# ZhenghaoFei/visual_odom

Measured on NVIDIA H100. Metric: stereo frames/sec at 1241x376, 2000 feats; LK kernel HBM GB/s vs roofline, higher is better.
Workload: dtype u8/i32 fixed point + f32 (LK), f64 (pose)

## Files before the change

visual_odom_b200/csrc/batch.cu:

```cuda
#include "ctx.h"
#include <string.h>
#include <algorithm>

__global__ void k_pack_counts(vo_unit_result_dev* res, const int* n_pts, const int* n_det, const int* n3, const int* n5,
                              int n_units, int detect)
{
    const int u = blockIdx.x * blockDim.x + threadIdx.x;
    if (u >= n_units) return;
    res[u].n_features = n_pts[u];
    res[u].n_detected = detect ? n_det[u] : 0;
    res[u].n_tracked = n3[u];
    res[u].n_valid = n5[u];
}

#define VO_OUT_BYTES_PER_SLOT (4 * sizeof(float2) + sizeof(int) + sizeof(float3) + sizeof(int))
__global__ void k_pack_outputs(uint8_t* __restrict__ out, size_t stride, int per, const float2* __restrict__ valid4, size_t cs,
                               const int* __restrict__ idx5, const float3* __restrict__ X, const int* __restrict__ inliers,
                               const int* __restrict__ n5, const vo_unit_result_dev* __restrict__ res, int cap)
{
    const int u = blockIdx.x;
    const int nv = min(n5[u], per), ni = min(res[u].n_inliers, per);
    float2* o4 = reinterpret_cast<float2*>(out + (size_t)u * stride);
    int* ok = reinterpret_cast<int*>(o4 + 4 * (size_t)per);
    float* oX = reinterpret_cast<float*>(ok + per);
// ... 43 lines not shown
    uint8_t* h = nullptr;
    const cudaError_t e = cudaMallocHost(&h, stride * ctx->units + 256);
    if (e != cudaSuccess) { cudaFree(q); VO_CUDA_CHECK(e); }
    if (ctx->h_out) {
        const int nu = ctx->out_units < ctx->units ? ctx->out_units : ctx->units;
        const int m = ctx->out_per < per ? ctx->out_per : per;
        for (int u = 0; u < nu; u++) {
            const PackedUnit a = packed_unit(ctx->h_out + (size_t)u * ctx->out_stride, ctx->out_per), b = packed_unit(h + (size_t)u * stride, per);
            for (int k = 0; k < 4; k++) memcpy(b.o4 + (size_t)k * per, a.o4 + (size_t)k * ctx->out_per, (size_t)m * sizeof(float2));
            memcpy(b.ok, a.ok, (size_t)m * sizeof(int));
            memcpy(b.oX, a.oX, (size_t)m * 3 * sizeof(float));
            memcpy(b.oi, a.oi, (size_t)m * sizeof(int));
        }
        cudaFreeHost(ctx->h_out);
    }
    ctx->h_out = h;
    if (ctx->d_out) {
        ctx->allocs.erase(std::find(ctx->allocs.begin(), ctx->allocs.end(), (void*)ctx->d_out));
        cudaFree(ctx->d_out);
    }
    ctx->allocs.push_back(q);
    ctx->d_out = (uint8_t*)q;
    ctx->out_units = ctx->units; ctx->out_per = per; ctx->out_stride = stride;
    return VO_OK;
}

extern "C" int vo_batch_configure(vo_ctx* ctx, int w, int h, int n_units, const float P_l[12], const float P_r[12])
{
    if (!ctx) return VO_E_INVALID;
    if (!P_l || !P_r || n_units <= 0) { vo_set_error(ctx, "bad argument"); return VO_E_INVALID; }
    VO_CUDA_CHECK(cudaSetDevice(ctx->device));
    int rc = vo_claim_buffers(ctx, "vo_batch_configure");
    if (rc) return rc;
    if ((rc = vo_ensure_state(ctx, w, h, n_units, 4))) return rc;
    vo_set_calibration(ctx, P_l, P_r);
    ctx->batch_units = n_units;
    ctx->batch_uploaded = 0;
    ctx->slot_pts.assign(n_units, 0);
    return VO_OK;
}

static int upload_range(vo_ctx* ctx, const vo_unit* units, int u0, int n, size_t pitch, cudaStream_t st, bool detect, int src0 = -1)
{
    if (src0 < 0) src0 = u0;
    const int w = ctx->w, h = ctx->h, cap = ctx->cap;
    const int total = ctx->batch_units;
    double* h_tprev = (double*)ctx->h_pinned;
    int* h_cnt = (int*)(h_tprev + 3 * (size_t)total);
    for (int u = u0; u < u0 + n; u++) {
        const vo_unit& U = units[u - u0 + src0];
        const uint8_t* imgs[4] = {U.l0, U.r0, U.l1, U.r1};
        for (int k = 0; k < 4; k++) {
            uint8_t* dst = ctx->d_raw + ((size_t)u * 4 + k) * w * h;
            if (pitch == (size_t)w) VO_CUDA_CHECK(cudaMemcpyAsync(dst, imgs[k], (size_t)w * h, cudaMemcpyHostToDevice, st));
            else VO_CUDA_CHECK(cudaMemcpy2DAsync(dst, w, imgs[k], pitch, w, h, cudaMemcpyHostToDevice, st));
        }
        if (!detect && U.n_pts > 0)
            VO_CUDA_CHECK(cudaMemcpyAsync(ctx->d_pts_in + (size_t)u * cap, U.pts, (size_t)U.n_pts * sizeof(float2),
                                          cudaMemcpyHostToDevice, st));
        h_cnt[u] = U.n_pts;
        ctx->slot_pts[u] = U.n_pts;
        for (int k = 0; k < 3; k++) h_tprev[3 * u + k] = U.t_prev[k];
    }
    VO_CUDA_CHECK(cudaMemcpyAsync(ctx->d_tprev + 3 * (size_t)u0, h_tprev + 3 * (size_t)u0, (size_t)n * 3 * sizeof(double),
                                  cudaMemcpyHostToDevice, st));
    VO_CUDA_CHECK(cudaMemcpyAsync((detect ? ctx->d_want : ctx->d_npts) + u0, h_cnt + u0, (size_t)n * sizeof(int),
                                  cudaMemcpyHostToDevice, st));
    return VO_OK;
}

static int validate_units(vo_ctx* ctx, const vo_unit* units, int n_units, size_t pitch, bool* detect_out, int* max_pts_out = nullptr)
{
    if (!ctx || !units) return VO_E_INVALID;
    if (n_units <= 0 || n_units > ctx->batch_units) { vo_set_error(ctx, "n_units=%d outside the configured batch (%d)", n_units, ctx->batch_units); return VO_E_INVALID; }
    if (pitch < (size_t)ctx->w) { vo_set_error(ctx, "pitch %zu < width %d", pitch, ctx->w); return VO_E_INVALID; }
    const bool detect = (units[0].pts == nullptr);
    int max_pts = 0;
    for (int u = 0; u < n_units; u++) {
        const vo_unit& U = units[u];
        if (!U.l0 || !U.r0 || !U.l1 || !U.r1) { vo_set_error(ctx, "unit %d: null image", u); return VO_E_INVALID; }
        if ((U.pts == nullptr) != detect) { vo_set_error(ctx, "units must all carry features or all request detection"); return VO_E_INVALID; }
        if (U.n_pts < 0 || U.n_pts > ctx->cap) { vo_set_error(ctx, "unit %d: n_pts=%d outside [0,%d]", u, U.n_pts, ctx->cap); return VO_E_CAPACITY; }
        if (U.n_pts > max_pts) max_pts = U.n_pts;
    }
    *detect_out = detect;
    if (max_pts_out) *max_pts_out = max_pts;
    const size_t bytes = (size_t)ctx->batch_units * (3 * sizeof(double) + sizeof(int) + sizeof(vo_unit_result_dev)) + 256;
    return vo_ensure_pinned(ctx, bytes);
}

static vo_unit_result_dev* pinned_results(vo_ctx* ctx)
{
    char* p = (char*)ctx->h_pinned + (size_t)ctx->batch_units * (3 * sizeof(double) + sizeof(int));
    p = (char*)(((uintptr_t)p + 63) & ~(uintptr_t)63);
    return (vo_unit_result_dev*)p;
}

extern "C" int vo_batch_upload(vo_ctx* ctx, const vo_unit* units, int n_units, size_t pitch)
{
    bool detect;
    int rc = validate_units(ctx, units, n_units, pitch, &detect);
    if (rc) return rc;
    VO_CUDA_CHECK(cudaSetDevice(ctx->device));
    if ((rc = vo_claim_buffers(ctx, "vo_batch_upload", true))) return rc;
    if ((rc = vo_drain_pending(ctx))) return rc;
    VO_CUDA_CHECK(cudaStreamSynchronize(ctx->stream));
    if ((rc = upload_range(ctx, units, 0, n_units, pitch, ctx->stream, detect))) return rc;
    ctx->batch_uploaded = n_units;
    ctx->batch_detect = detect;
    return VO_OK;
}

static int ensure_side_streams(vo_ctx* ctx)
{
    if (ctx->fork_ev) return VO_OK;
    VO_CUDA_CHECK(cudaEventCreateWithFlags(&ctx->fork_ev, cudaEventDisableTiming));
    for (int c = 0; c < VO_LANES; c++) {
        VO_CUDA_CHECK(cudaStreamCreateWithFlags(&ctx->side_stream[c], cudaStreamNonBlocking));
        VO_CUDA_CHECK(cudaEventCreateWithFlags(&ctx->join_ev[c], cudaEventDisableTiming));
    }
    return VO_OK;
}

static int ensure_hi_streams(vo_ctx* ctx)
{
    if (ctx->hi_stream[0]) return VO_OK;
    int lo = 0, hi = 0;
    VO_CUDA_CHECK(cudaDeviceGetStreamPriorityRange(&lo, &hi));
    for (int c = 0; c < VO_LANES; c++) {
        VO_CUDA_CHECK(cudaStreamCreateWithPriority(&ctx->hi_stream[c], cudaStreamNonBlocking, hi));
        for (int k = 0; k < 4; k++) VO_CUDA_CHECK(cudaEventCreateWithFlags(&ctx->hi_ev[c][k], cudaEventDisableTiming));
    }
    return VO_OK;
}

static int run_range_launch(vo_ctx* ctx, const View& v)
{
    ctx->imgs_per_unit = 4;
    int rc;
    int c = -1;
    for (int k = 0; k < VO_LANES; k++) if (ctx->side_stream[k] && v.s == ctx->side_stream[k]) c = k;
    const bool part = ctx->part_on && c >= 0;
    const bool prio = !part && ctx->use_priorities && c >= 0;
    View h = v, lk = v;
    cudaEvent_t* ev = nullptr;
    if (part) {
        h.s = ctx->part_hp_stream[c]; lk.s = ctx->part_lk_stream[c]; ev = ctx->part_ev[c];
    } else if (prio) {
        if ((rc = ensure_hi_streams(ctx))) return rc;
        h.s = ctx->hi_stream[c]; ev = ctx->hi_ev[c];
    }
    View pre = h;
    if (part && ctx->part_pre_with_lk) pre.s = lk.s;
    if (ev) {
        VO_CUDA_CHECK(cudaEventRecord(ev[0], v.s));
        VO_CUDA_CHECK(cudaStreamWaitEvent(pre.s, ev[0], 0));
        if (pre.s != h.s) VO_CUDA_CHECK(cudaStreamWaitEvent(h.s, ev[0], 0));
    }
    if (ctx->batch_detect) {
        if ((rc = vo_run_fast(ctx, pre, 0, false))) return rc;
        if ((rc = vo_run_select(ctx, pre))) return rc;
    }
    if ((rc = vo_run_pyramid(ctx, v.u0 * ctx->imgs_per_unit, v.n * ctx->imgs_per_unit, pre.s))) return rc;
    if (ev && pre.s != lk.s) {
        VO_CUDA_CHECK(cudaEventRecord(ev[1], pre.s));
        VO_CUDA_CHECK(cudaStreamWaitEvent(lk.s, ev[1], 0));
    }
    const int ip[4] = {0, 1, 3, 2}, in[4] = {1, 3, 2, 0};
    ctx->lk_per_unit = range_bound(ctx, v.u0, v.n);
    rc = vo_run_lk_ring(ctx, lk, 4, ip, in, false);
    ctx->lk_per_unit = 0;
    if (rc) return rc;
    if (ev) {
        VO_CUDA_CHECK(cudaEventRecord(ev[2], lk.s));
        VO_CUDA_CHECK(cudaStreamWaitEvent(h.s, ev[2], 0));
    }
    if ((rc = vo_run_filter(ctx, h, false))) return rc;
    const size_t cs = (size_t)ctx->units * ctx->cap;
    if ((rc = vo_run_triangulate(ctx, h, ctx->d_valid4, ctx->d_valid4 + cs, ctx->d_n5))) return rc;
    float K9[9] = {ctx->P_l[0], ctx->P_l[1], ctx->P_l[2], ctx->P_l[4], ctx->P_l[5], ctx->P_l[6], ctx->P_l[8], ctx->P_l[9], ctx->P_l[10]};
    if ((rc = vo_run_pnp(ctx, h, ctx->d_valid4 + 2 * cs, ctx->d_n5, K9))) return rc;
    k_pack_counts<<<(v.n + 63) / 64, 64, 0, h.s>>>(ctx->d_results + v.u0, ctx->d_npts + v.u0, ctx->d_ndet + v.u0, ctx->d_n3 + v.u0,
                                                  ctx->d_n5 + v.u0, v.n, ctx->batch_detect ? 1 : 0);
    ctx->launches += 1;
    VO_CUDA_CHECK(cudaGetLastError());
    if (ev) {
        VO_CUDA_CHECK(cudaEventRecord(ev[3], h.s));
        VO_CUDA_CHECK(cudaStreamWaitEvent(v.s, ev[3], 0));
    }
    return VO_OK;
}

static int run_range(vo_ctx* ctx, const View& v)
{
    bool on_side = false;
    for (int k = 0; k < VO_LANES; k++) on_side = on_side || (ctx->side_stream[k] && v.s == ctx->side_stream[k]);
    if (!ctx->use_graphs || ((ctx->use_priorities || ctx->part_on) && on_side && !ctx->batch_graphs)) return run_range_launch(ctx, v);
    const int max_pts = range_bound(ctx, v.u0, v.n);
    for (auto& g : ctx->graphs)
        if (g.u0 == v.u0 && g.n == v.n && g.detect == ctx->batch_detect && g.tma == ctx->lk_use_tma && g.s == v.s && g.max_pts == max_pts) {
            VO_CUDA_CHECK(cudaGraphLaunch(g.exec, v.s));
            ctx->launches += g.launches;
            return VO_OK;
        }
    const bool timing = ctx->lk_timing;
    const long long before = ctx->launches;
    ctx->lk_timing = false;
    cudaGraph_t graph = nullptr;
    VO_CUDA_CHECK(cudaStreamBeginCapture(v.s, cudaStreamCaptureModeThreadLocal));
    int rc = run_range_launch(ctx, v);
    cudaError_t e = cudaStreamEndCapture(v.s, &graph);
    ctx->lk_timing = timing;
    if (rc) { if (graph) cudaGraphDestroy(graph); return rc; }
    VO_CUDA_CHECK(e);
    vo_ctx::RangeGraph g;
    g.u0 = v.u0; g.n = v.n; g.detect = ctx->batch_detect; g.tma = ctx->lk_use_tma; g.s = v.s; g.max_pts = max_pts;
    g.launches = ctx->launches - before;
    VO_CUDA_CHECK(cudaGraphInstantiate(&g.exec, graph, 0));
    cudaGraphDestroy(graph);
    ctx->graphs.push_back(g);
    VO_CUDA_CHECK(cudaGraphLaunch(g.exec, v.s));
    return VO_OK;
}

extern "C" int vo_batch_run(vo_ctx* ctx)
{
    if (!ctx) return VO_E_INVALID;
    const int units = ctx->batch_uploaded;
    if (units <= 0) { vo_set_error(ctx, "vo_batch_run: nothing uploaded"); return VO_E_INVALID; }
    if (!ctx->have_P) { vo_set_error(ctx, "vo_batch_run: projection matrices not set"); return VO_E_INVALID; }
    { int rcc = vo_claim_buffers(ctx, "vo_batch_run"); if (rcc) return rcc; }
    VO_CUDA_CHECK(cudaSetDevice(ctx->device));
    if (units < 2 || ctx->batch_streams < 2) return run_range(ctx, View{0, units, ctx->stream});
    int rc = ensure_side_streams(ctx);
    if (rc) return rc;
    VO_CUDA_CHECK(cudaEventRecord(ctx->fork_ev, ctx->stream));
    const int half = (units + 1) / 2;
    for (int c = 0; c < 2; c++) {
        const int u0 = c ? half : 0, n = c ? units - half : half;
        cudaStream_t st = ctx->side_stream[c];
        VO_CUDA_CHECK(cudaStreamWaitEvent(st, ctx->fork_ev, 0));
        if ((rc = run_range(ctx, View{u0, n, st}))) return rc;
        VO_CUDA_CHECK(cudaEventRecord(ctx->join_ev[c], st));
        VO_CUDA_CHECK(cudaStreamWaitEvent(ctx->stream, ctx->join_ev[c], 0));
    }
    return VO_OK;
}

extern "C" int vo_batch_download(vo_ctx* ctx, vo_unit_result* results, int n_units)
{
    if (!ctx || !results) return VO_E_INVALID;
    if (n_units <= 0 || n_units > ctx->batch_uploaded) { vo_set_error(ctx, "n_units=%d outside the resident batch (%d)", n_units, ctx->batch_uploaded); return VO_E_INVALID; }
    static_assert(sizeof(vo_unit_result) == sizeof(vo_unit_result_dev), "result record layout");
    VO_CUDA_CHECK(cudaSetDevice(ctx->device));
    VO_CUDA_CHECK(cudaMemcpyAsync(results, ctx->d_results, (size_t)n_units * sizeof(vo_unit_result), cudaMemcpyDeviceToHost, ctx->stream));
    VO_CUDA_CHECK(cudaStreamSynchronize(ctx->stream));
    return VO_OK;
}

extern "C" int vo_frame_batch(vo_ctx* ctx, const vo_unit* units, int n_units, size_t pitch, vo_unit_result* results)
{
    bool detect;
    int rc = validate_units(ctx, units, n_units, pitch, &detect);
    if (rc) return rc;
    if (!results) return VO_E_INVALID;
    if (!ctx->have_P) { vo_set_error(ctx, "vo_frame_batch: projection matrices not set"); return VO_E_INVALID; }
    VO_CUDA_CHECK(cudaSetDevice(ctx->device));
    if ((rc = vo_claim_buffers(ctx, "vo_frame_batch", true))) return rc;
    if ((rc = vo_drain_pending(ctx))) return rc;
    VO_CUDA_CHECK(cudaStreamSynchronize(ctx->stream));
    ctx->batch_uploaded = n_units; ctx->batch_detect = detect;
    vo_unit_result_dev* h_res = pinned_results(ctx);
    const int nchunks = (n_units >= 2 && ctx->batch_streams >= 2) ? 2 : 1;
    if (nchunks == 1) {
        if ((rc = upload_range(ctx, units, 0, n_units, pitch, ctx->stream, detect))) return rc;
        if ((rc = run_range(ctx, View{0, n_units, ctx->stream}))) return rc;
        VO_CUDA_CHECK(cudaMemcpyAsync(h_res, ctx->d_results, (size_t)n_units * sizeof(vo_unit_result_dev), cudaMemcpyDeviceToHost, ctx->stream));
    } else {
        if ((rc = ensure_side_streams(ctx))) return rc;
        VO_CUDA_CHECK(cudaEventRecord(ctx->fork_ev, ctx->stream));
        const int half = (n_units + 1) / 2;
        for (int c = 0; c < 2; c++) {
            const int u0 = c ? half : 0, n = c ? n_units - half : half;
            cudaStream_t st = ctx->side_stream[c];
            VO_CUDA_CHECK(cudaStreamWaitEvent(st, ctx->fork_ev, 0));
            if ((rc = upload_range(ctx, units, u0, n, pitch, st, detect))) return rc;
            if ((rc = run_range(ctx, View{u0, n, st}))) return rc;
            VO_CUDA_CHECK(cudaMemcpyAsync(h_res + u0, ctx->d_results + u0, (size_t)n * sizeof(vo_unit_result_dev), cudaMemcpyDeviceToHost, st));
            VO_CUDA_CHECK(cudaEventRecord(ctx->join_ev[c], st));
            VO_CUDA_CHECK(cudaStreamWaitEvent(ctx->stream, ctx->join_ev[c], 0));
        }
    }
    VO_CUDA_CHECK(cudaStreamSynchronize(ctx->stream));
    memcpy(results, h_res, (size_t)n_units * sizeof(vo_unit_result));
    return VO_OK;
}

extern "C" int vo_batch_submit(vo_ctx* ctx, const vo_unit* units, int first_unit, int n_units, size_t pitch)
{
    if (!ctx) return VO_E_INVALID;
    if (first_unit < 0 || n_units <= 0 || first_unit + n_units > ctx->batch_units) {
        vo_set_error(ctx, "vo_batch_submit: slots [%d, %d) outside the configured batch (%d)", first_unit, first_unit + n_units, ctx->batch_units);
        return VO_E_INVALID;
    }
    if (!ctx->have_P) { vo_set_error(ctx, "vo_batch_submit: projection matrices not set"); return VO_E_INVALID; }
    { int rcc = vo_claim_buffers(ctx, "vo_batch_submit", true); if (rcc) return rcc; }
    for (auto& p : ctx->pending)
        if (p.active && first_unit < p.u0 + p.n && p.u0 < first_unit + n_units) {
            vo_set_error(ctx, "vo_batch_submit: slots [%d, %d) overlap a submission that has not been waited for", first_unit, first_unit + n_units);
            return VO_E_INVALID;
        }
    bool detect = ctx->batch_detect; int max_pts = 0;
    int rc;
    if (units) {
        if ((rc = validate_units(ctx, units, n_units, pitch, &detect, &max_pts))) return rc;
    } else {
        if (ctx->batch_uploaded < first_unit + n_units) {
            vo_set_error(ctx, "vo_batch_submit: units == NULL but slots [%d, %d) were never uploaded", first_unit, first_unit + n_units);
            return VO_E_INVALID;
// ... 110 lines not shown
```

visual_odom_b200/csrc/ctx.cu:

```cuda
#include "ctx.h"
#include <string.h>
#include <stdlib.h>

void vo_set_error(vo_ctx* ctx, const char* fmt, ...)
{
    if (!ctx) return;
    va_list ap;
    va_start(ap, fmt);
    vsnprintf(ctx->err, sizeof(ctx->err), fmt, ap);
    va_end(ap);
}

extern "C" void vo_default_params(vo_params* p)
{
    p->fast_threshold = 20;
    p->fast_nonmax = 1;
    p->lk_win = 21;
    p->lk_max_level = 3;
    p->lk_max_iters = 30;
    p->lk_epsilon = 0.01;
    p->lk_min_eig = 0.001;
    p->circ_threshold = 0;
    p->pnp_iterations = 500;
    p->pnp_reproj_error = 0.5f;
// ... 39 lines not shown
    VO_CUDA_CHECK(cudaStreamCreateWithFlags(&ctx->own_stream, cudaStreamNonBlocking));
    ctx->stream = ctx->own_stream;
    VO_CUDA_CHECK(vo_lk_prepare());
    ctx->cap = ctx->p.max_features;
    VO_CUDA_CHECK(cudaMalloc(&ctx->d_lk_queue, LK_QUEUES * 2 * sizeof(int)));
    VO_CUDA_CHECK(cudaMemset(ctx->d_lk_queue, 0, LK_QUEUES * 2 * sizeof(int)));
    {
        const char* st = getenv("VO_LK_STAGING");
        ctx->lk_use_tma = !(st && strcmp(st, "ldg") == 0);
        const char* sp = getenv("VO_LK_SPAN");
        if (sp) ctx->lk_span = atoi(sp);
        const char* pt = getenv("VO_SM_PARTITION");
        if (pt && atoi(pt) == 0) ctx->part_auto = false;
    }
    return VO_OK;
}

extern "C" void vo_destroy(vo_ctx* ctx)
{
    if (!ctx) return;
    cudaSetDevice(ctx->device);
    vo_drain_pending(ctx);
    if (ctx->stream) cudaStreamSynchronize(ctx->stream);
    vo_dist_shutdown(ctx);
    vo_partition_destroy(ctx);
    vo_free_state(ctx);
    for (cudaEvent_t e : ctx->ev_pool) cudaEventDestroy(e);
    for (auto& p : ctx->pending) if (p.done) cudaEventDestroy(p.done);
    for (int k = 0; k < 2; k++) {
        if (ctx->seq_front_ev[k]) cudaEventDestroy(ctx->seq_front_ev[k]);
        if (ctx->seq_back_ev[k]) cudaEventDestroy(ctx->seq_back_ev[k]);
    }
    if (ctx->fork_ev) cudaEventDestroy(ctx->fork_ev);
    for (int c = 0; c < VO_LANES; c++) {
        if (ctx->join_ev[c]) cudaEventDestroy(ctx->join_ev[c]);
        if (ctx->side_stream[c]) cudaStreamDestroy(ctx->side_stream[c]);
        if (ctx->hi_stream[c]) cudaStreamDestroy(ctx->hi_stream[c]);
        for (int k = 0; k < 4; k++) if (ctx->hi_ev[c][k]) cudaEventDestroy(ctx->hi_ev[c][k]);
    }
    if (ctx->h_pinned) cudaFreeHost(ctx->h_pinned);
    if (ctx->d_bgr) cudaFree(ctx->d_bgr);
    if (ctx->d_lk_queue) cudaFree(ctx->d_lk_queue);
    if (ctx->d_ess) cudaFree(ctx->d_ess);
    if (ctx->h_out) cudaFreeHost(ctx->h_out);
    if (ctx->own_stream) cudaStreamDestroy(ctx->own_stream);
    delete ctx;
}

extern "C" const char* vo_last_error(const vo_ctx* ctx) { return ctx ? ctx->err : "null context"; }

extern "C" int vo_set_stream(vo_ctx* ctx, void* s)
{
    if (!ctx) return VO_E_INVALID;
    VO_CUDA_CHECK(cudaStreamSynchronize(ctx->stream));
    ctx->stream = s ? (cudaStream_t)s : ctx->own_stream;
    return VO_OK;
}

extern "C" int vo_sync(vo_ctx* ctx)
{
    if (!ctx) return VO_E_INVALID;
    VO_CUDA_CHECK(cudaStreamSynchronize(ctx->stream));
    return VO_OK;
}

extern "C" int vo_set_option(vo_ctx* ctx, const char* key, double value)
{
    if (!ctx || !key) return VO_E_INVALID;
    if (strcmp(key, "batch_streams") == 0) { ctx->batch_streams = value >= 2 ? 2 : 1; return VO_OK; }
    if (strcmp(key, "lk_staging") == 0) { ctx->lk_use_tma = !(value >= 1); return VO_OK; }
    if (strcmp(key, "lk_ctas_per_sm") == 0) { ctx->lk_ctas_per_sm = (int)value; vo_drop_graphs(ctx); return VO_OK; }
    if (strcmp(key, "batch_outputs") == 0) { ctx->batch_outputs = value >= 1; vo_drop_graphs(ctx); return VO_OK; }
    if (strcmp(key, "sm_partition") == 0) {
        ctx->part_pre_with_lk = value < 0;
        ctx->part_auto = false;
        return vo_partition_enable(ctx, value < 0 ? (int)-value : (int)value);
    }
    if (strcmp(key, "lk_quota") == 0) { ctx->lk_quota = (int)value; vo_drop_graphs(ctx); return VO_OK; }
    if (strcmp(key, "lk_span") == 0) { ctx->lk_span = (int)value; vo_drop_graphs(ctx); return VO_OK; }
    if (strcmp(key, "graphs") == 0) { ctx->use_graphs = value >= 1; return VO_OK; }
    if (strcmp(key, "batch_graphs") == 0) { ctx->batch_graphs = value >= 1; return VO_OK; }
    if (strcmp(key, "priorities") == 0) { ctx->use_priorities = value >= 1; vo_drop_graphs(ctx); return VO_OK; }
    vo_set_error(ctx, "unknown option %s", key);
    return VO_E_INVALID;
}

extern "C" long long vo_kernel_launches(const vo_ctx* ctx) { return ctx ? ctx->launches : 0; }

extern "C" int vo_lk_kernel_time(vo_ctx* ctx, double* ms_total, long long* n, int reset)
{
    if (!ctx) return VO_E_INVALID;
    VO_CUDA_CHECK(cudaStreamSynchronize(ctx->stream));
    for (size_t i = 0; i + 1 < ctx->ev_used; i += 2) {
        float ms = 0.f;
        VO_CUDA_CHECK(cudaEventElapsedTime(&ms, ctx->ev_pool[i], ctx->ev_pool[i + 1]));
        ctx->lk_ms += ms;
        ctx->lk_n++;
    }
    ctx->ev_used = 0;
    if (ms_total) *ms_total = ctx->lk_ms;
    if (n) *n = ctx->lk_n;
    if (reset) { ctx->lk_ms = 0.0; ctx->lk_n = 0; }
    return VO_OK;
}

int vo_ensure_pinned(vo_ctx* ctx, size_t bytes)
{
    if (bytes <= ctx->h_pinned_bytes) return VO_OK;
    if (ctx->h_pinned) { cudaFreeHost(ctx->h_pinned); ctx->h_pinned = nullptr; ctx->h_pinned_bytes = 0; }
    VO_CUDA_CHECK(cudaMallocHost(&ctx->h_pinned, bytes));
    ctx->h_pinned_bytes = bytes;
    return VO_OK;
}

int vo_claim_buffers(vo_ctx* ctx, const char* who, bool allow_pending_batches)
{
    if (ctx->seq_inflight > 0) {
        vo_set_error(ctx, "%s: %d frame(s) submitted with vo_seq_submit have not been waited for (this call would overwrite their buffers)", who, ctx->seq_inflight);
        return VO_E_INVALID;
    }
    if (!allow_pending_batches)
        for (auto& p : ctx->pending)
            if (p.active) {
                vo_set_error(ctx, "%s: the vo_batch_submit submission of slots [%d, %d) has not been waited for", who, p.u0, p.u0 + p.n);
                return VO_E_INVALID;
            }
    ctx->seq_active = false;
    return VO_OK;
}

typedef CUresult (*PFN_cuDeviceGet)(CUdevice*, int);
typedef CUresult (*PFN_cuDeviceGetDevResource)(CUdevice, CUdevResource*, CUdevResourceType);
typedef CUresult (*PFN_cuDevSmResourceSplitByCount)(CUdevResource*, unsigned int*, const CUdevResource*, CUdevResource*, unsigned int, unsigned int);
typedef CUresult (*PFN_cuDevResourceGenerateDesc)(CUdevResourceDesc*, CUdevResource*, unsigned int);
typedef CUresult (*PFN_cuGreenCtxCreate)(CUgreenCtx*, CUdevResourceDesc, CUdevice, unsigned int);
typedef CUresult (*PFN_cuGreenCtxStreamCreate)(CUstream*, CUgreenCtx, unsigned int, int);
typedef CUresult (*PFN_cuGreenCtxDestroy)(CUgreenCtx);

template <typename F>
static bool drv(const char* name, F* fn)
{
    void* p = nullptr;
    cudaDriverEntryPointQueryResult q;
    if (cudaGetDriverEntryPoint(name, &p, cudaEnableDefault, &q) != cudaSuccess || q != cudaDriverEntryPointSuccess || !p) return false;
    *fn = (F)p;
    return true;
}

void vo_partition_destroy(vo_ctx* ctx)
{
    for (int c = 0; c < VO_LANES; c++) {
        if (ctx->part_lk_stream[c]) cudaStreamDestroy(ctx->part_lk_stream[c]);
        if (ctx->part_hp_stream[c]) cudaStreamDestroy(ctx->part_hp_stream[c]);
        ctx->part_lk_stream[c] = ctx->part_hp_stream[c] = nullptr;
        for (int k = 0; k < 4; k++) if (ctx->part_ev[c][k]) { cudaEventDestroy(ctx->part_ev[c][k]); ctx->part_ev[c][k] = nullptr; }
    }
    PFN_cuGreenCtxDestroy destroy = nullptr;
    if (drv("cuGreenCtxDestroy", &destroy))
        for (int k = 0; k < 2; k++) if (ctx->part_gctx[k]) destroy((CUgreenCtx)ctx->part_gctx[k]);
    ctx->part_gctx[0] = ctx->part_gctx[1] = nullptr;
    ctx->part_on = false; ctx->part_helper_sms = ctx->part_lk_sms = 0;
}

int vo_partition_enable(vo_ctx* ctx, int helper_sms)
{
    VO_CUDA_CHECK(cudaSetDevice(ctx->device));
    int rc = vo_drain_pending(ctx);
    if (rc) return rc;
    VO_CUDA_CHECK(cudaDeviceSynchronize());
    vo_drop_graphs(ctx);
    vo_partition_destroy(ctx);
    if (helper_sms <= 0) return VO_OK;
    PFN_cuDeviceGet dget; PFN_cuDeviceGetDevResource getres; PFN_cuDevSmResourceSplitByCount split;
    PFN_cuDevResourceGenerateDesc gendesc; PFN_cuGreenCtxCreate create; PFN_cuGreenCtxStreamCreate screate;
    if (!drv("cuDeviceGet", &dget) || !drv("cuDeviceGetDevResource", &getres) || !drv("cuDevSmResourceSplitByCount", &split) ||
        !drv("cuDevResourceGenerateDesc", &gendesc) || !drv("cuGreenCtxCreate", &create) || !drv("cuGreenCtxStreamCreate", &screate)) {
        vo_set_error(ctx, "sm_partition: this driver has no green-context API");
        return VO_E_UNSUPPORTED;
    }
    CUdevice dev;
    CUdevResource all, part[1], rest;
    unsigned int nb = 1;
    CUresult r;
    if ((r = dget(&dev, ctx->device)) != CUDA_SUCCESS || (r = getres(dev, &all, CU_DEV_RESOURCE_TYPE_SM)) != CUDA_SUCCESS ||
        (r = split(part, &nb, &all, &rest, 0, (unsigned)helper_sms)) != CUDA_SUCCESS || nb != 1) {
        vo_set_error(ctx, "sm_partition: splitting off %d SMs failed (driver error %d)", helper_sms, (int)r);
        return VO_E_UNSUPPORTED;
    }
    CUdevResource* rs[2] = {&part[0], &rest};
    for (int k = 0; k < 2; k++) {
        CUdevResourceDesc desc;
        CUgreenCtx g;
        if ((r = gendesc(&desc, rs[k], 1)) != CUDA_SUCCESS || (r = create(&g, desc, dev, CU_GREEN_CTX_DEFAULT_STREAM)) != CUDA_SUCCESS) {
            vo_set_error(ctx, "sm_partition: cuGreenCtxCreate failed (driver error %d)", (int)r);
            vo_partition_destroy(ctx);
            return VO_E_UNSUPPORTED;
        }
        ctx->part_gctx[k] = g;
    }
    ctx->part_helper_sms = (int)part[0].sm.smCount; ctx->part_lk_sms = (int)rest.sm.smCount;
    for (int c = 0; c < VO_LANES; c++) {
        CUstream a, b;
        if ((r = screate(&a, (CUgreenCtx)ctx->part_gctx[0], CU_STREAM_NON_BLOCKING, 0)) != CUDA_SUCCESS ||
            (r = screate(&b, (CUgreenCtx)ctx->part_gctx[1], CU_STREAM_NON_BLOCKING, 0)) != CUDA_SUCCESS) {
            vo_set_error(ctx, "sm_partition: cuGreenCtxStreamCreate failed (driver error %d)", (int)r);
            vo_partition_destroy(ctx);
            return VO_E_UNSUPPORTED;
        }
        ctx->part_hp_stream[c] = (cudaStream_t)a; ctx->part_lk_stream[c] = (cudaStream_t)b;
        for (int k = 0; k < 4; k++) VO_CUDA_CHECK(cudaEventCreateWithFlags(&ctx->part_ev[c][k], cudaEventDisableTiming));
    }
    ctx->part_on = true;
    return VO_OK;
}

int vo_drain_pending(vo_ctx* ctx)
{
    for (auto& p : ctx->pending)
        if (p.active) {
            VO_CUDA_CHECK(cudaEventSynchronize(p.done));
            p.active = false;
        }
    if (ctx->seq_inflight > 0 && ctx->side_stream[0]) VO_CUDA_CHECK(cudaStreamSynchronize(ctx->side_stream[0]));
    return VO_OK;
}

void vo_drop_graphs(vo_ctx* ctx)
{
    for (auto& g : ctx->graphs) cudaGraphExecDestroy(g.exec);
    ctx->graphs.clear();
}

void vo_set_calibration(vo_ctx* ctx, const float P_l[12], const float P_r[12])
{
    const bool same = ctx->have_P && memcmp(ctx->P_l, P_l, 12 * sizeof(float)) == 0 && memcmp(ctx->P_r, P_r, 12 * sizeof(float)) == 0;
    if (same) return;
    vo_drop_graphs(ctx);
    memcpy(ctx->P_l, P_l, 12 * sizeof(float));
    memcpy(ctx->P_r, P_r, 12 * sizeof(float));
    ctx->have_P = true;
}

void vo_free_state(vo_ctx* ctx)
{
    vo_drop_graphs(ctx);
    for (void* p : ctx->allocs) cudaFree(p);
    ctx->allocs.clear();
    ctx->d_out = nullptr; ctx->out_stride = 0; ctx->out_per = 0;
    ctx->w = ctx->h = ctx->units = 0;
}

template <typename T>
static cudaError_t dalloc(vo_ctx* ctx, T** p, size_t count)
{
    void* q = nullptr;
    cudaError_t e = cudaMalloc(&q, count * sizeof(T) + 256);
    if (e == cudaSuccess) { ctx->allocs.push_back(q); *p = (T*)q; }
    return e;
}

typedef CUresult (*PFN_encodeTiled)(CUtensorMap*, CUtensorMapDataType, cuuint32_t, void*, const cuuint64_t*,
                                    const cuuint64_t*, const cuuint32_t*, const cuuint32_t*, CUtensorMapInterleave,
                                    CUtensorMapSwizzle, CUtensorMapL2promotion, CUtensorMapFloatOOBfill);

static int encode_maps(vo_ctx* ctx)
{
    void* fn = nullptr;
    cudaDriverEntryPointQueryResult qres;
    VO_CUDA_CHECK(cudaGetDriverEntryPoint("cuTensorMapEncodeTiled", &fn, cudaEnableDefault, &qres));
    if (!fn || qres != cudaDriverEntryPointSuccess) {
        vo_set_error(ctx, "cuTensorMapEncodeTiled not available from the driver");
        return VO_E_CUDA;
    }
    PFN_encodeTiled enc = (PFN_encodeTiled)fn;
    const int n_img = ctx->units * 4;
    for (int l = 0; l < ctx->pg.nlevels; l++) {
        const LevelGeom& g = ctx->pg.lv[l];
        {
            cuuint64_t dims[3] = {(cuuint64_t)g.pitch, (cuuint64_t)g.hp, (cuuint64_t)n_img};
            cuuint64_t strides[2] = {(cuuint64_t)g.pitch, (cuuint64_t)g.plane};
            cuuint32_t box_i[3] = {48, 22, 1}, box_j[3] = {48, 32, 1};
            cuuint32_t estr[3] = {1, 1, 1};
            CUresult r = enc(&ctx->maps.img_i[l], CU_TENSOR_MAP_DATA_TYPE_UINT8, 3, g.img, dims, strides, box_i, estr,
                             CU_TENSOR_MAP_INTERLEAVE_NONE, CU_TENSOR_MAP_SWIZZLE_NONE,
                             CU_TENSOR_MAP_L2_PROMOTION_NONE, CU_TENSOR_MAP_FLOAT_OOB_FILL_NONE);
            if (r == CUDA_SUCCESS)
                r = enc(&ctx->maps.img_j[l], CU_TENSOR_MAP_DATA_TYPE_UINT8, 3, g.img, dims, strides, box_j, estr,
                        CU_TENSOR_MAP_INTERLEAVE_NONE, CU_TENSOR_MAP_SWIZZLE_NONE,
                        CU_TENSOR_MAP_L2_PROMOTION_NONE, CU_TENSOR_MAP_FLOAT_OOB_FILL_NONE);
            if (r != CUDA_SUCCESS) { vo_set_error(ctx, "cuTensorMapEncodeTiled(u8 level %d) failed: %d", l, (int)r); return VO_E_CUDA; }
        }
        {
            cuuint64_t dims[3] = {(cuuint64_t)g.pitch, (cuuint64_t)g.hp, (cuuint64_t)n_img};
            cuuint64_t strides[2] = {(cuuint64_t)g.pitch * 4, (cuuint64_t)g.plane * 4};
            cuuint32_t box[3] = {28, 22, 1};
            cuuint32_t estr[3] = {1, 1, 1};
            CUresult r = enc(&ctx->maps.der[l], CU_TENSOR_MAP_DATA_TYPE_UINT32, 3, g.der, dims, strides, box, estr,
                             CU_TENSOR_MAP_INTERLEAVE_NONE, CU_TENSOR_MAP_SWIZZLE_NONE,
                             CU_TENSOR_MAP_L2_PROMOTION_NONE, CU_TENSOR_MAP_FLOAT_OOB_FILL_NONE);
            if (r != CUDA_SUCCESS) { vo_set_error(ctx, "cuTensorMapEncodeTiled(deriv level %d) failed: %d", l, (int)r); return VO_E_CUDA; }
        }
    }
    return VO_OK;
}

int vo_ensure_state(vo_ctx* ctx, int w, int h, int units, int )
{
    if (w <= 0 || h <= 0 || units <= 0) { vo_set_error(ctx, "bad geometry %dx%d units=%d", w, h, units); return VO_E_INVALID; }
    if (ctx->w == w && ctx->h == h && ctx->units >= units) return VO_OK;
    VO_CUDA_CHECK(cudaSetDevice(ctx->device));
    { int drc = vo_drain_pending(ctx); if (drc) return drc; }
    VO_CUDA_CHECK(cudaStreamSynchronize(ctx->stream));
    vo_free_state(ctx);
    const int n_img = units * 4;
    const int cap = ctx->cap;
    PyrGeom& pg = ctx->pg;
    memset(&pg, 0, sizeof(pg));
    int cw = w, ch = h;
    for (int l = 0; l <= ctx->p.lk_max_level; l++) {
        if (l > 0) {
            int nw = (cw + 1) / 2, nh = (ch + 1) / 2;
            if (nw <= VO_WIN || nh <= VO_WIN) break;
            cw = nw; ch = nh;
        }
        LevelGeom& g = pg.lv[l];
        g.w = cw; g.h = ch;
        g.pitch = ((cw + 2 * VO_PAD) + 63) / 64 * 64;
        g.hp = ch + 2 * VO_PAD;
        g.plane = (size_t)g.pitch * g.hp;
        VO_CUDA_CHECK(dalloc(ctx, &g.img, g.plane * n_img));
        VO_CUDA_CHECK(dalloc(ctx, &g.der, g.plane * n_img));
        VO_CUDA_CHECK(cudaMemsetAsync(g.img, 0, g.plane * n_img, ctx->stream));
        VO_CUDA_CHECK(cudaMemsetAsync(g.der, 0, g.plane * n_img * sizeof(uint32_t), ctx->stream));
        pg.nlevels = l + 1;
    }
    pg.n_img = n_img;
    VO_CUDA_CHECK(dalloc(ctx, &ctx->d_raw, (size_t)n_img * w * h));
    VO_CUDA_CHECK(dalloc(ctx, &ctx->d_raw_tab, (size_t)n_img));
    {
        std::vector<const uint8_t*> tab(n_img);
        for (int i = 0; i < n_img; i++) tab[i] = ctx->d_raw + (size_t)i * w * h;
        VO_CUDA_CHECK(cudaMemcpyAsync(ctx->d_raw_tab, tab.data(), n_img * sizeof(uint8_t*), cudaMemcpyHostToDevice, ctx->stream));
        VO_CUDA_CHECK(cudaStreamSynchronize(ctx->stream));
    }
    const size_t uc = (size_t)units * cap;
    VO_CUDA_CHECK(dalloc(ctx, &ctx->d_pts_in, uc));
    VO_CUDA_CHECK(dalloc(ctx, &ctx->d_npts, (size_t)units));
    VO_CUDA_CHECK(dalloc(ctx, &ctx->d_pts_out, 4 * uc));
    VO_CUDA_CHECK(dalloc(ctx, &ctx->d_status, 4 * uc));
    VO_CUDA_CHECK(dalloc(ctx, &ctx->d_err, 4 * uc));
    VO_CUDA_CHECK(dalloc(ctx, &ctx->d_lk_progress, uc));
    VO_CUDA_CHECK(cudaMemsetAsync(ctx->d_lk_progress, 0, uc * sizeof(int), ctx->stream));
    VO_CUDA_CHECK(dalloc(ctx, &ctx->d_ages_in, uc));
    VO_CUDA_CHECK(dalloc(ctx, &ctx->d_ages_out, uc));
    VO_CUDA_CHECK(dalloc(ctx, &ctx->d_kept5, 5 * uc));
    VO_CUDA_CHECK(dalloc(ctx, &ctx->d_idx3, uc));
    VO_CUDA_CHECK(dalloc(ctx, &ctx->d_n3, (size_t)units));
    VO_CUDA_CHECK(dalloc(ctx, &ctx->d_valid4, 4 * uc));
    VO_CUDA_CHECK(dalloc(ctx, &ctx->d_idx5, uc));
    VO_CUDA_CHECK(dalloc(ctx, &ctx->d_n5, (size_t)units));
    {
        const long iw = w > 6 ? w - 6 : 0, ih = h > 6 ? h - 6 : 0;
        const long bound = ctx->p.fast_nonmax ? ((iw + 1) / 2) * ((ih + 1) / 2) : iw * ih;
// ... 216 lines not shown
```

visual_odom_b200/csrc/ctx.h:

```cpp
#pragma once
#include "common.cuh"
#include "lk_ring.h"
#include "filter.h"
#include "fast.h"
#include "pnp.h"
#include "seq.h"
#include "ess.h"
#include "../../include/vo_b200.h"
#include <vector>
#include <stdarg.h>
#define LK_QUEUES 32
#define VO_DIST_BUCKET 4
#define VO_DIST_NB 4
#define VO_LANES 3

struct vo_ctx {
    int device = 0;
    cudaStream_t own_stream = nullptr, stream = nullptr;
    vo_params p;
    char err[1024] = {0};
    long long launches = 0;
    int sm_count = 0;

    int w = 0, h = 0;
    int units = 0;
    int imgs_per_unit = 4;
    int cap = 0;
    PyrGeom pg;
    LkMaps maps;
    bool have_P = false;
    float P_l[12], P_r[12];

    uint8_t* d_raw = nullptr;
    const uint8_t** d_raw_tab = nullptr;
    float2* d_pts_in = nullptr;
    int* d_npts = nullptr;
    float2* d_pts_out = nullptr;
    uint8_t* d_status = nullptr;
    float* d_err = nullptr;
    int* d_ages_in = nullptr;
    int* d_ages_out = nullptr;
    float2* d_kept5 = nullptr;
    int* d_idx3 = nullptr;
    int* d_n3 = nullptr;
    float2* d_valid4 = nullptr;
    int* d_idx5 = nullptr;
    int* d_n5 = nullptr;
    uint8_t* d_score = nullptr;
    uint16_t* d_rowbuf = nullptr;
    int* d_rowcount = nullptr;
    int* d_rowoff = nullptr;
    int* d_ndet = nullptr;
    float2* d_corners = nullptr;
    float* d_resp = nullptr;
    int* d_want = nullptr;
    int corner_cap = 0;
    float3* d_X = nullptr;
    double* d_tprev = nullptr;
    PnpState* d_pnp_state = nullptr;
    int* d_subsets = nullptr;
    double* d_models = nullptr;
    int* d_counts = nullptr;
    int* d_inliers = nullptr;
    vo_unit_result_dev* d_results = nullptr;
    float2* d_feat_pts = nullptr;
    int* d_feat_ages = nullptr;
    int* d_feat_cnt = nullptr;
    int* d_bucket = nullptr;
    int* d_seq_err = nullptr;
    int feat_cap = 0, bucket_cap = 4096;
    bool seq_active = false;
    int seq_slot = 0;
    int seq_inflight = 0;
    long long seq_submitted = 0;
    int seq_channels[2] = {1, 1};
    cudaEvent_t seq_front_ev[2] = {nullptr, nullptr}, seq_back_ev[2] = {nullptr, nullptr};
    long long seq_frames = 0;
    double seq_pose[16] = {1,0,0,0, 0,1,0,0, 0,0,1,0, 0,0,0,1};
    uint8_t* d_bgr = nullptr;
    size_t bgr_bytes = 0;
    bool part_on = false;
    bool part_auto = true;
    bool part_pre_with_lk = false;
    int part_helper_sms = 0, part_lk_sms = 0;
    void* part_gctx[2] = {nullptr, nullptr};
    cudaStream_t part_lk_stream[VO_LANES] = {};
    cudaStream_t part_hp_stream[VO_LANES] = {};
    cudaEvent_t part_ev[VO_LANES][4] = {};
    void* dist_comm = nullptr;
    int dist_rank = 0, dist_world = 1;
    cudaStream_t dist_stream = nullptr, dist_snap_stream = nullptr;
    struct DistBucket { void* d = nullptr; void* h = nullptr; cudaEvent_t done = nullptr; int fill = 0, unwaited = 0, n_units = 0; bool flushed = false; };
    struct DistStep { int bucket = 0, index = 0; };
    DistBucket dist_bk[VO_DIST_NB];
    DistStep dist_steps[2 * VO_DIST_DEPTH];
    int dist_cur = 0;
    cudaEvent_t dist_ev_read = nullptr, dist_ev_fork = nullptr;
    size_t dist_bytes = 0;
    long long dist_head = 0, dist_tail = 0;
    void* d_ess = nullptr;
    int ess_cap = 0;
    std::vector<void*> allocs;

    void* h_pinned = nullptr;
    size_t h_pinned_bytes = 0;

    std::vector<cudaEvent_t> ev_pool;
    size_t ev_used = 0;
    double lk_ms = 0.0;
    long long lk_n = 0;
    bool lk_timing = true;
    bool lk_use_tma = true;
    int lk_ctas_per_sm = 0;
    int lk_quota = 0;
    int lk_span = 0;
    int* d_lk_progress = nullptr;
    int lk_per_unit = 0;
    int* d_lk_queue = nullptr;
    std::vector<cudaStream_t> lk_queue_streams;

    int batch_units = 0;
    int batch_uploaded = 0;
    bool batch_detect = false;
    int batch_streams = 2;
    bool use_graphs = true;
    struct RangeGraph { int u0, n; bool detect, tma; cudaStream_t s; int max_pts; cudaGraphExec_t exec; long long launches; };
    std::vector<RangeGraph> graphs;
    std::vector<int> slot_pts;
    cudaStream_t hi_stream[VO_LANES] = {};
    cudaEvent_t hi_ev[VO_LANES][4] = {};
    bool use_priorities = true;
    bool batch_graphs = false;
    cudaStream_t side_stream[VO_LANES] = {};
    cudaEvent_t fork_ev = nullptr, join_ev[VO_LANES] = {};
    struct Pending { int u0 = 0, n = 0; bool active = false; cudaEvent_t done = nullptr; };
    std::vector<Pending> pending;
    bool batch_outputs = false;
    uint8_t* d_out = nullptr;
    uint8_t* h_out = nullptr;
    size_t out_stride = 0;
    int out_per = 0, out_units = 0;
    unsigned submit_count = 0;
};

void vo_set_error(vo_ctx* ctx, const char* fmt, ...);
int vo_ensure_state(vo_ctx* ctx, int w, int h, int units, int imgs_per_unit);
void vo_free_state(vo_ctx* ctx);
void vo_drop_graphs(vo_ctx* ctx);
void vo_set_calibration(vo_ctx* ctx, const float P_l[12], const float P_r[12]);
int vo_drain_pending(vo_ctx* ctx);
int vo_partition_enable(vo_ctx* ctx, int helper_sms);
void vo_partition_destroy(vo_ctx* ctx);
int vo_dist_order_after_gathers(vo_ctx* ctx, cudaStream_t st);
void vo_dist_shutdown(vo_ctx* ctx);
int vo_claim_buffers(vo_ctx* ctx, const char* who, bool allow_pending_batches = false);
int vo_ensure_pinned(vo_ctx* ctx, size_t bytes);
int vo_ensure_bgr(vo_ctx* ctx, size_t bytes);
int vo_launch_bgr_to_gray(const uint8_t* d_bgr, size_t pitch, size_t img_stride_in, uint8_t* d_gray, size_t img_stride_out,
                          int w, int h, int n_img, cudaStream_t s);
struct View { int u0, n; cudaStream_t s; int plane0 = -1; };
int vo_run_lk(vo_ctx* ctx, const View& v, int ncalls, const int* img_prev, const int* img_next, bool want_err);
int vo_run_pyramid(vo_ctx* ctx, int plane0, int nplanes, cudaStream_t s);
int vo_run_lk_ring(vo_ctx* ctx, const View& v, int ncalls, const int* img_prev, const int* img_next, bool want_err);
int vo_run_filter(vo_ctx* ctx, const View& v, bool with_ages);
int vo_run_fast(vo_ctx* ctx, const View& v, int plane_in_unit, bool want_resp);
int vo_run_select(vo_ctx* ctx, const View& v);
int vo_run_triangulate(vo_ctx* ctx, const View& v, const float2* pts_l, const float2* pts_r, const int* n, float4* X4 = nullptr);
int vo_run_pnp(vo_ctx* ctx, const View& v, const float2* pts2d, const int* n, const float* K9);
```

visual_odom_b200/csrc/fast.cu:

```cuda
#include "common.cuh"
#include "fast.h"

__global__ void __launch_bounds__(256) k_fast_score(const uint8_t* const* __restrict__ img_tab, int img_stride_idx,
                                                    int w, int h, int pitch, int threshold, int nonmax,
                                                    uint8_t* __restrict__ score, size_t score_plane)
{
    constexpr int ring_dx[16] = {0, 1, 2, 3, 3, 3, 2, 1, 0, -1, -2, -3, -3, -3, -2, -1};
    constexpr int ring_dy[16] = {3, 3, 2, 1, 0, -1, -2, -3, -3, -3, -2, -1, 0, 1, 2, 3};
    const int unit = blockIdx.z;
    const uint8_t* __restrict__ img = img_tab[unit * img_stride_idx];
    uint8_t* __restrict__ sc = score + (size_t)unit * score_plane;
    const int x = blockIdx.x * 32 + (threadIdx.x & 31);
    const int y = blockIdx.y * 8 + (threadIdx.x >> 5);
    if (x >= w || y >= h) return;
    int result = 0;
    if (x >= 3 && x < w - 3 && y >= 3 && y < h - 3) {
        const uint8_t* p = img + (size_t)y * pitch + x;
        const int v = p[0];
        float d[16];
        unsigned hi = 0, lo = 0;
#pragma unroll
        for (int k = 0; k < 16; k++) {
            const int r = p[ring_dy[k] * pitch + ring_dx[k]];
            d[k] = (float)(v - r);
            hi |= (unsigned)(r > v + threshold) << k;
            lo |= (unsigned)(r < v - threshold) << k;
        }
        unsigned mh = hi | (hi << 16), ml = lo | (lo << 16);
        mh &= mh >> 1; mh &= mh >> 2; mh &= mh >> 4; mh &= mh >> 1;
        ml &= ml >> 1; ml &= ml >> 2; ml &= ml >> 4; ml &= ml >> 1;
        if (mh | ml) {
            float mn[16], mx[16];
#pragma unroll
            for (int k = 0; k < 16; k++) { mn[k] = fminf(d[k], d[(k + 1) & 15]); mx[k] = fmaxf(d[k], d[(k + 1) & 15]); }
            float mn4[16], mx4[16];
#pragma unroll
            for (int k = 0; k < 16; k++) { mn4[k] = fminf(mn[k], mn[(k + 2) & 15]); mx4[k] = fmaxf(mx[k], mx[(k + 2) & 15]); }
            float A = -1000.f, B = 1000.f;
#pragma unroll
            for (int k = 0; k < 16; k++) {
                const float a8 = fminf(mn4[k], mn4[(k + 4) & 15]);
                const float b8 = fmaxf(mx4[k], mx4[(k + 4) & 15]);
                A = fmaxf(A, fminf(a8, d[(k + 8) & 15]));
                B = fminf(B, fmaxf(b8, d[(k + 8) & 15]));
            }
            result = max(threshold, (int)fmaxf(A, -B)) - 1;
            if (!nonmax) result = 1;
        }
    }
    sc[(size_t)y * w + x] = (uint8_t)result;
}

#define NMS_T 256
#define NMS_NC 8
__global__ void __launch_bounds__(NMS_T) k_fast_nms_row(const uint8_t* __restrict__ score, size_t score_plane, int w, int h,
                                                        int nonmax, uint16_t* __restrict__ rowbuf, int rowcap,
                                                        int* __restrict__ rowcount)
{
    const int y = blockIdx.x, unit = blockIdx.y;
    const uint8_t* __restrict__ sc = score + (size_t)unit * score_plane;
    uint16_t* __restrict__ out = rowbuf + ((size_t)unit * h + y) * rowcap;
    __shared__ uint8_t rows[3][NMS_T * NMS_NC + 2];
    __shared__ int wcnt[NMS_NC * (NMS_T / 32)];
    __shared__ int base;
    if (y < 3 || y >= h - 3) {
        if (threadIdx.x == 0) rowcount[unit * h + y] = 0;
        return;
    }
    if (threadIdx.x == 0) base = 0;
    const int lane = threadIdx.x & 31, warp = threadIdx.x >> 5;
    constexpr int NW = NMS_T / 32, SPAN = NMS_T * NMS_NC;
    for (int x0 = 0; x0 < w; x0 += SPAN) {
        for (int i = threadIdx.x; i < SPAN + 2; i += NMS_T) {
            const int x = x0 - 1 + i;
            const bool in = (x >= 0 && x < w);
            rows[0][i] = in ? sc[(size_t)(y - 1) * w + x] : 0;
            rows[1][i] = in ? sc[(size_t)y * w + x] : 0;
            rows[2][i] = in ? sc[(size_t)(y + 1) * w + x] : 0;
        }
        __syncthreads();
        unsigned bal[NMS_NC];
#pragma unroll
        for (int c = 0; c < NMS_NC; c++) {
            const int x = x0 + c * NMS_T + threadIdx.x, i = c * NMS_T + threadIdx.x + 1;
            bool keep = false;
            if (x < w) {
                const int s = rows[1][i];
                if (s > 0) {
                    keep = !nonmax ||
                           (s > rows[1][i - 1] && s > rows[1][i + 1] && s > rows[0][i - 1] && s > rows[0][i] &&
                            s > rows[0][i + 1] && s > rows[2][i - 1] && s > rows[2][i] && s > rows[2][i + 1]);
                }
            }
            bal[c] = __ballot_sync(0xffffffffu, keep);
            if (lane == 0) wcnt[c * NW + warp] = __popc(bal[c]);
        }
        __syncthreads();
        int carry_total = 0;
        if (threadIdx.x < NMS_NC * NW) {
            const int v = wcnt[threadIdx.x];
            int incl = v;
#pragma unroll
            for (int d = 1; d < 32; d <<= 1) {
                const int o = __shfl_up_sync(0xffffffffu, incl, d);
                if (lane >= d) incl += o;
            }
            carry_total = incl;
            wcnt[threadIdx.x] = incl - v;
        }
        __shared__ int w0_total, pass_total;
        if (threadIdx.x == 31) w0_total = carry_total;
        __syncthreads();
        if (threadIdx.x >= 32 && threadIdx.x < NMS_NC * NW) wcnt[threadIdx.x] += w0_total;
        if (threadIdx.x == NMS_NC * NW - 1) pass_total = carry_total + w0_total;
        __syncthreads();
        const int b0 = base;
#pragma unroll
        for (int c = 0; c < NMS_NC; c++) {
            if ((bal[c] >> lane) & 1u) {
                const int o = b0 + wcnt[c * NW + warp] + __popc(bal[c] & ((1u << lane) - 1u));
                if (o < rowcap) out[o] = (uint16_t)(x0 + c * NMS_T + threadIdx.x);
            }
        }
        __syncthreads();
        if (threadIdx.x == 0) base = b0 + pass_total;
        __syncthreads();
    }
    if (threadIdx.x == 0) rowcount[unit * h + y] = base < rowcap ? base : rowcap;
}

__global__ void __launch_bounds__(1024) k_fast_scan(const int* __restrict__ rowcount, int h, int* __restrict__ rowoff,
                                                    int* __restrict__ n_det)
{
    const int unit = blockIdx.x;
    const int* rc = rowcount + unit * h;
    int* ro = rowoff + unit * h;
    __shared__ int wsum[32];
    __shared__ int carry;
    if (threadIdx.x == 0) carry = 0;
    __syncthreads();
    const int lane = threadIdx.x & 31, warp = threadIdx.x >> 5;
    for (int y0 = 0; y0 < h; y0 += 1024) {
        const int y = y0 + threadIdx.x;
        int v = (y < h) ? rc[y] : 0;
        int incl = v;
#pragma unroll
        for (int d = 1; d < 32; d <<= 1) {
            int o = __shfl_up_sync(0xffffffffu, incl, d);
            if (lane >= d) incl += o;
        }
        if (lane == 31) wsum[warp] = incl;
        __syncthreads();
        int woff = carry;
        for (int k = 0; k < warp; k++) woff += wsum[k];
        if (y < h) ro[y] = woff + incl - v;
        __syncthreads();
        if (threadIdx.x == 0) {
            int t = 0;
            for (int k = 0; k < 32; k++) t += wsum[k];
            carry += t;
        }
        __syncthreads();
    }
    if (threadIdx.x == 0) n_det[unit] = carry;
}

__global__ void __launch_bounds__(128) k_fast_gather(const uint16_t* __restrict__ rowbuf, int rowcap,
                                                     const int* __restrict__ rowcount, const int* __restrict__ rowoff,
                                                     int h, const uint8_t* __restrict__ score, size_t score_plane, int w,
                                                     int nonmax, float2* __restrict__ out, float* __restrict__ resp, int cap)
{
    const int y = blockIdx.x, unit = blockIdx.y;
    const int n = rowcount[unit * h + y], off = rowoff[unit * h + y];
    const uint16_t* src = rowbuf + ((size_t)unit * h + y) * rowcap;
    for (int i = threadIdx.x; i < n; i += blockDim.x) {
        const int o = off + i;
        if (o < cap) {
            const int x = src[i];
            out[(size_t)unit * cap + o] = make_float2((float)x, (float)y);
            if (resp)
                resp[(size_t)unit * cap + o] = nonmax ? (float)score[(size_t)unit * score_plane + (size_t)y * w + x] : 0.f;
        }
    }
}

__global__ void k_select_stride(const float2* __restrict__ corners, int corner_cap, const int* __restrict__ n_det,
                                const int* __restrict__ want, float2* __restrict__ pts, int cap, int* __restrict__ n_pts)
{
    const int unit = blockIdx.y;
    int m = n_det[unit];
    if (m > corner_cap) m = corner_cap;
    int n = want[unit];
    if (n > cap) n = cap;
    if (n > m) n = m;
    const int i = blockIdx.x * blockDim.x + threadIdx.x;
    if (i == 0) n_pts[unit] = n;
    if (i >= n) return;
    const long idx = (n > 1) ? ((long)i * (m - 1)) / (n - 1) : 0;
    pts[(size_t)unit * cap + i] = corners[(size_t)unit * corner_cap + idx];
// ... 23 lines not shown
```

Baseline: 4148.

## Run pyramid on its own green-context stream and pack FAST score into half2

New measurement: 4220 (median of 6 runs). +1.7%, better.

```diff
diff --git a/visual_odom_b200/csrc/batch.cu b/visual_odom_b200/csrc/batch.cu
--- a/visual_odom_b200/csrc/batch.cu
+++ b/visual_odom_b200/csrc/batch.cu
@@ -219,19 +219,25 @@
     }
     View pre = h;
     if (part && ctx->part_pre_with_lk) pre.s = lk.s;
+    const cudaStream_t pyr = part ? ctx->part_pyr_stream[c] : pre.s;
     if (ev) {
         VO_CUDA_CHECK(cudaEventRecord(ev[0], v.s));
         VO_CUDA_CHECK(cudaStreamWaitEvent(pre.s, ev[0], 0));
         if (pre.s != h.s) VO_CUDA_CHECK(cudaStreamWaitEvent(h.s, ev[0], 0));
+        if (pyr != pre.s) VO_CUDA_CHECK(cudaStreamWaitEvent(pyr, ev[0], 0));
     }
     if (ctx->batch_detect) {
         if ((rc = vo_run_fast(ctx, pre, 0, false))) return rc;
         if ((rc = vo_run_select(ctx, pre))) return rc;
     }
-    if ((rc = vo_run_pyramid(ctx, v.u0 * ctx->imgs_per_unit, v.n * ctx->imgs_per_unit, pre.s))) return rc;
+    if ((rc = vo_run_pyramid(ctx, v.u0 * ctx->imgs_per_unit, v.n * ctx->imgs_per_unit, pyr))) return rc;
     if (ev && pre.s != lk.s) {
         VO_CUDA_CHECK(cudaEventRecord(ev[1], pre.s));
         VO_CUDA_CHECK(cudaStreamWaitEvent(lk.s, ev[1], 0));
+    }
+    if (pyr != pre.s) {
+        VO_CUDA_CHECK(cudaEventRecord(ev[4], pyr));
+        VO_CUDA_CHECK(cudaStreamWaitEvent(lk.s, ev[4], 0));
     }
     const int ip[4] = {0, 1, 3, 2}, in[4] = {1, 3, 2, 0};
     ctx->lk_per_unit = range_bound(ctx, v.u0, v.n);
diff --git a/visual_odom_b200/csrc/ctx.cu b/visual_odom_b200/csrc/ctx.cu
--- a/visual_odom_b200/csrc/ctx.cu
+++ b/visual_odom_b200/csrc/ctx.cu
@@ -215,8 +215,9 @@
     for (int c = 0; c < VO_LANES; c++) {
         if (ctx->part_lk_stream[c]) cudaStreamDestroy(ctx->part_lk_stream[c]);
         if (ctx->part_hp_stream[c]) cudaStreamDestroy(ctx->part_hp_stream[c]);
-        ctx->part_lk_stream[c] = ctx->part_hp_stream[c] = nullptr;
-        for (int k = 0; k < 4; k++) if (ctx->part_ev[c][k]) { cudaEventDestroy(ctx->part_ev[c][k]); ctx->part_ev[c][k] = nullptr; }
+        if (ctx->part_pyr_stream[c]) cudaStreamDestroy(ctx->part_pyr_stream[c]);
+        ctx->part_lk_stream[c] = ctx->part_hp_stream[c] = ctx->part_pyr_stream[c] = nullptr;
+        for (int k = 0; k < 5; k++) if (ctx->part_ev[c][k]) { cudaEventDestroy(ctx->part_ev[c][k]); ctx->part_ev[c][k] = nullptr; }
     }
     PFN_cuGreenCtxDestroy destroy = nullptr;
     if (drv("cuGreenCtxDestroy", &destroy))
@@ -263,15 +264,17 @@
     }
     ctx->part_helper_sms = (int)part[0].sm.smCount; ctx->part_lk_sms = (int)rest.sm.smCount;
     for (int c = 0; c < VO_LANES; c++) {
-        CUstream a, b;
-        if ((r = screate(&a, (CUgreenCtx)ctx->part_gctx[0], CU_STREAM_NON_BLOCKING, 0)) != CUDA_SUCCESS ||
-            (r = screate(&b, (CUgreenCtx)ctx->part_gctx[1], CU_STREAM_NON_BLOCKING, 0)) != CUDA_SUCCESS) {
+        CUstream a = nullptr, b = nullptr, p = nullptr;
+        r = screate(&a, (CUgreenCtx)ctx->part_gctx[0], CU_STREAM_NON_BLOCKING, 0);
+        if (r == CUDA_SUCCESS) r = screate(&b, (CUgreenCtx)ctx->part_gctx[1], CU_STREAM_NON_BLOCKING, 0);
+        if (r == CUDA_SUCCESS) r = screate(&p, (CUgreenCtx)ctx->part_gctx[ctx->part_pre_with_lk ? 1 : 0], CU_STREAM_NON_BLOCKING, 0);
+        ctx->part_hp_stream[c] = (cudaStream_t)a; ctx->part_lk_stream[c] = (cudaStream_t)b; ctx->part_pyr_stream[c] = (cudaStream_t)p;
+        if (r != CUDA_SUCCESS) {
             vo_set_error(ctx, "sm_partition: cuGreenCtxStreamCreate failed (driver error %d)", (int)r);
             vo_partition_destroy(ctx);
             return VO_E_UNSUPPORTED;
         }
-        ctx->part_hp_stream[c] = (cudaStream_t)a; ctx->part_lk_stream[c] = (cudaStream_t)b;
-        for (int k = 0; k < 4; k++) VO_CUDA_CHECK(cudaEventCreateWithFlags(&ctx->part_ev[c][k], cudaEventDisableTiming));
+        for (int k = 0; k < 5; k++) VO_CUDA_CHECK(cudaEventCreateWithFlags(&ctx->part_ev[c][k], cudaEventDisableTiming));
     }
     ctx->part_on = true;
     return VO_OK;
diff --git a/visual_odom_b200/csrc/ctx.h b/visual_odom_b200/csrc/ctx.h
--- a/visual_odom_b200/csrc/ctx.h
+++ b/visual_odom_b200/csrc/ctx.h
@@ -86,7 +86,8 @@
     void* part_gctx[2] = {nullptr, nullptr};
     cudaStream_t part_lk_stream[VO_LANES] = {};
     cudaStream_t part_hp_stream[VO_LANES] = {};
-    cudaEvent_t part_ev[VO_LANES][4] = {};
+    cudaStream_t part_pyr_stream[VO_LANES] = {};
+    cudaEvent_t part_ev[VO_LANES][5] = {};
     void* dist_comm = nullptr;
     int dist_rank = 0, dist_world = 1;
     cudaStream_t dist_stream = nullptr, dist_snap_stream = nullptr;
diff --git a/visual_odom_b200/csrc/fast.cu b/visual_odom_b200/csrc/fast.cu
--- a/visual_odom_b200/csrc/fast.cu
+++ b/visual_odom_b200/csrc/fast.cu
@@ -1,5 +1,6 @@
 #include "common.cuh"
 #include "fast.h"
+#include <cuda_fp16.h>
 
 __global__ void __launch_bounds__(256) k_fast_score(const uint8_t* const* __restrict__ img_tab, int img_stride_idx,
                                                     int w, int h, int pitch, int threshold, int nonmax,
@@ -16,12 +17,12 @@
     int result = 0;
     if (x >= 3 && x < w - 3 && y >= 3 && y < h - 3) {
         const uint8_t* p = img + (size_t)y * pitch + x;
-        const int v = p[0];
+        const int v = __ldg(p);
         float d[16];
         unsigned hi = 0, lo = 0;
 #pragma unroll
         for (int k = 0; k < 16; k++) {
-            const int r = p[ring_dy[k] * pitch + ring_dx[k]];
+            const int r = __ldg(p + ring_dy[k] * pitch + ring_dx[k]);
             d[k] = (float)(v - r);
             hi |= (unsigned)(r > v + threshold) << k;
             lo |= (unsigned)(r < v - threshold) << k;
@@ -30,21 +31,19 @@
         mh &= mh >> 1; mh &= mh >> 2; mh &= mh >> 4; mh &= mh >> 1;
         ml &= ml >> 1; ml &= ml >> 2; ml &= ml >> 4; ml &= ml >> 1;
         if (mh | ml) {
-            float mn[16], mx[16];
-#pragma unroll
-            for (int k = 0; k < 16; k++) { mn[k] = fminf(d[k], d[(k + 1) & 15]); mx[k] = fmaxf(d[k], d[(k + 1) & 15]); }
-            float mn4[16], mx4[16];
-#pragma unroll
-            for (int k = 0; k < 16; k++) { mn4[k] = fminf(mn[k], mn[(k + 2) & 15]); mx4[k] = fmaxf(mx[k], mx[(k + 2) & 15]); }
-            float A = -1000.f, B = 1000.f;
-#pragma unroll
-            for (int k = 0; k < 16; k++) {
-                const float a8 = fminf(mn4[k], mn4[(k + 4) & 15]);
-                const float b8 = fmaxf(mx4[k], mx4[(k + 4) & 15]);
-                A = fmaxf(A, fminf(a8, d[(k + 8) & 15]));
-                B = fminf(B, fmaxf(b8, d[(k + 8) & 15]));
-            }
-            result = max(threshold, (int)fmaxf(A, -B)) - 1;
+            __half2 e[16];
+#pragma unroll
+            for (int k = 0; k < 16; k++) e[k] = __floats2half2_rn(d[k], -d[k]);
+            __half2 m2[16];
+#pragma unroll
+            for (int k = 0; k < 16; k++) m2[k] = __hmin2(e[k], e[(k + 1) & 15]);
+            __half2 m4[16];
+#pragma unroll
+            for (int k = 0; k < 16; k++) m4[k] = __hmin2(m2[k], m2[(k + 2) & 15]);
+            __half2 S = __floats2half2_rn(-1000.f, -1000.f);
+#pragma unroll
+            for (int k = 0; k < 16; k++) S = __hmax2(S, __hmin2(__hmin2(m4[k], m4[(k + 4) & 15]), e[(k + 8) & 15]));
+            result = max(threshold, (int)fmaxf(__low2float(S), __high2float(S))) - 1;
             if (!nonmax) result = 1;
         }
     }
```
